# JayKickliter/Multirate.jl

Measured on AMD Instinct MI355X. Metric: Msamples/s in (Float32, 147//160, 24*147 taps) + achieved HBM GB/s vs roofline, higher is better.
Workload: dtype f32

## Files before the change

### multirate.jl_amd/csrc/api.hip

```cpp
#include <algorithm>
#include <cmath>
#include <chrono>
#include <cstdlib>
#include <cstring>
#include <mutex>
#include <numeric>
#include <unordered_map>

#include "mrhip_filter.h"

namespace mrhip {

bool plan_farrow_wave(const FarrowArgs &a);
hipError_t launch_farrow_wave(const TypeKey &tk, bool fused, const FarrowArgs &a, hipStream_t s, const char **kname, int num_cus);

thread_local LaunchEvents g_launch_events;
static thread_local std::string g_last_error;

void set_error(const std::string &msg) { g_last_error = msg; }

namespace {
struct OccKey { const void *fn; int dev; bool operator==(const OccKey &o) const { return fn == o.fn && dev == o.dev; } };
struct OccKeyHash { size_t operator()(const OccKey &k) const { return std::hash<const void *>()(k.fn) ^ (static_cast<size_t>(k.dev) * 0x9e3779b97f4a7c15ull); } };
struct OccEntry { unsigned block = 0; size_t lds = ~static_cast<size_t>(0), attr = 0; int per_cu = 0; };
// ... 1557 lines not shown
    }
    if (!same || stream_is_capturing(stream)) return single_calls();
    DeviceGuard guard(f0->device);
    if (!guard.ok) return fail(MRHIP_ERR_HIP, "hipSetDevice failed");
    const TypeKey tk = type_key(f0);
    const bool fused = f0->numerics == MRHIP_NUMERICS_FUSED;
    std::vector<CallPlan> plans(static_cast<size_t>(n));
    int64_t n_out_max = 0, nch_total = 0, x_len_max = 0;
    for (int i = 0; i < n; ++i) {
        mrhip_filter *f = filters[i];
        if (!f->mirror_valid)
            if (int rc = rec_pull(f)) return rc;
        plans[i] = plan_rational(f->kind, f->L, f->M, f->phiIdx, f->inputDeficit, x_len[i]);
        if (plans[i].n_out > y_capacity[i]) return fail(MRHIP_ERR_BUFFER_TOO_SMALL, "buffer is too small");
        n_out_max = std::max(n_out_max, plans[i].n_out);
        x_len_max = std::max(x_len_max, x_len[i]);
        nch_total += f->nch;
    }
    if (n_out_max < 1) return single_calls();
    PolyArgs a = poly_call_args(f0, x[0], y[0], x_len_max, n_out_max, x_len_max, false);
    a.n_out = n_out_max;
    a.u0 = 0; a.d0 = 1;
    a.nch = static_cast<int>(std::min<int64_t>(nch_total, 0x7fffffff));
    PairArgs pa;
    dim3 block;
    size_t lds = 0;
    const bool column = f0->L == 1;
    if (!(column ? plan_fir_stream(tk, a, f0->num_cus, &pa, &block, &lds) : plan_rational_opair(tk, fused, a, f0->num_cus, &pa, &block, &lds))) return single_calls();
    const size_t bytes = static_cast<size_t>(n) * sizeof(MultiDesc);
    if (int rc = multi_staging(f0, bytes)) return rc;
    MultiDesc *d = static_cast<MultiDesc *>(f0->multi_pin);
    unsigned steps_max = 0;
    for (int i = 0; i < n; ++i) {
        mrhip_filter *f = filters[i];
        if (int rc = adopt_stream(f, stream)) return rc;
        const CallPlan &p = plans[i];
        const int64_t spc = (p.n_out + pa.P - 1) / pa.P;
        if (spc * f->nch >= (1LL << 31)) return fail(MRHIP_ERR_INVALID_ARG, "stream too long for one launch");
        MultiDesc &m = d[i];
        m.x = x[i]; m.y = y[i]; m.hist = f->d_hist[f->hist_cur]; m.hist_new = f->d_hist[hist_other(f)]; m.taps = f->d_taps; m.rec = f->d_rec;
        m.x_stride = x_len[i]; m.y_stride = y_capacity[i]; m.x_len = x_len[i]; m.n_out = p.n_out;
        m.u0 = p.phi0 - 1; m.d0 = p.d0; m.phi_end = p.phi_end; m.d_end = p.d_end;
        m.steps_per_channel = static_cast<unsigned>(spc);
        m.total_steps = static_cast<unsigned>(spc * f->nch);
        m.spc_magic = step_magic(spc);
        m.nch = static_cast<int>(f->nch);
// ... 247 lines not shown
```

### multirate.jl_amd/csrc/kernels_rational_opair.hip

```cpp
#include <algorithm>
#include <cstdio>
#include <cstdlib>

#include "mrhip_internal.h"

namespace mrhip {

hipError_t launch_opair_f32_s0r(bool fused, int T, dim3 block, size_t lds, hipStream_t s, const PolyArgs &a, const PairArgs &pa, int num_cus);
hipError_t launch_opair_f32_s0c(bool fused, int T, dim3 block, size_t lds, hipStream_t s, const PolyArgs &a, const PairArgs &pa, int num_cus);
hipError_t launch_opair_f32_s1r(bool fused, int T, dim3 block, size_t lds, hipStream_t s, const PolyArgs &a, const PairArgs &pa, int num_cus);
hipError_t launch_opair_f32_s1c(bool fused, int T, dim3 block, size_t lds, hipStream_t s, const PolyArgs &a, const PairArgs &pa, int num_cus);
hipError_t launch_opair_f32_s0_long(int nc, bool fused, int T, dim3 block, size_t lds, hipStream_t s, const PolyArgs &a, const PairArgs &pa, int num_cus);
hipError_t launch_opair_f32_s1_long(int nc, bool fused, int T, dim3 block, size_t lds, hipStream_t s, const PolyArgs &a, const PairArgs &pa, int num_cus);
hipError_t launch_opair_f32_s2(int nc, bool fused, int T, dim3 block, size_t lds, hipStream_t s, const PolyArgs &a, const PairArgs &pa, int num_cus);
hipError_t launch_opair_f32_s3(int nc, bool fused, int T, dim3 block, size_t lds, hipStream_t s, const PolyArgs &a, const PairArgs &pa, int num_cus);
hipError_t launch_opair_f32_s4(int nc, bool fused, int T, dim3 block, size_t lds, hipStream_t s, const PolyArgs &a, const PairArgs &pa, int num_cus);
hipError_t launch_opair_f32_s5(int nc, bool fused, int T, dim3 block, size_t lds, hipStream_t s, const PolyArgs &a, const PairArgs &pa, int num_cus);
hipError_t launch_opair_wide_s0(bool x_f64, bool fused, int T, dim3 block, size_t lds, hipStream_t s, const PolyArgs &a, const PairArgs &pa, int num_cus);
hipError_t launch_opair_wide_s1(bool x_f64, bool fused, int T, dim3 block, size_t lds, hipStream_t s, const PolyArgs &a, const PairArgs &pa, int num_cus);
hipError_t launch_opair_cmix_s0(bool x_f64, bool fused, int T, dim3 block, size_t lds, hipStream_t s, const PolyArgs &a, const PairArgs &pa, int num_cus);
hipError_t launch_opair_cmix_s1(bool x_f64, bool fused, int T, dim3 block, size_t lds, hipStream_t s, const PolyArgs &a, const PairArgs &pa, int num_cus);

namespace {
constexpr int kOMaxThreads = 512;
#define opair_env_int(name, dflt) MRHIP_ENV_INT(name, dflt)
}

bool plan_rational_opair(const TypeKey &tk, bool fused, const PolyArgs &a, int num_cus, PairArgs *out, dim3 *block, size_t *lds, int force_wgpc)
{
    if (!opair_env_int("MRHIP_OPAIR", 1)) return false;
    if (tk.x_f64 && !tk.r_f64) return false;
    const int nc = tk.complex_x ? 2 : 1;
    const long long es = (tk.x_f64 ? 8 : 4) * nc;
#ifdef MRHIP_PS_FAST_BUILD
    if (a.T != 24 && !((a.T == 36 || a.T == 48) && !tk.complex_x) && !(!tk.r_f64 && (a.T == 36 || a.T == 48 || a.T == 56 || a.T == 64))) return false;
#endif
    if (a.T < 1 || a.T > (tk.r_f64 ? (tk.complex_x ? 32 : 48) : 64)) return false;
    if (a.L < 2 || a.M < 1 || a.zero_start_below > 0) return false;
    const int smin = static_cast<int>(a.M / a.L);
    if (smin > 5) return false;
    if (!opair_instantiated(fused, smin, a.T)) return false;
    if (smin >= 2 && (tk.r_f64 || a.T > 32)) return false;
    const int env_c = opair_env_int("MRHIP_OPAIR_C", 0), env_j = opair_env_int("MRHIP_OPAIR_J", 0), env_ns = opair_env_int("MRHIP_OPAIR_NS", 0);
    int best_c = 0;
    double best = -1.0;
    for (int pass = 0; pass < 2 && !best_c; ++pass)
        for (int c = 2; static_cast<long long>(c) * a.L / 2 <= kOMaxThreads && static_cast<long long>(c) * a.L <= 1024; c += 2) {
            const int lanes = static_cast<int>(static_cast<long long>(c) * a.L / 2);
            const int padded = (lanes + 63) / 64 * 64;
            if (pass == 0 && (padded < 192 || padded > 448)) continue;
            const double score = static_cast<double>(lanes) / padded * (padded < 192 ? 0.5 + 0.5 * padded / 192.0 : 1.0);
            if (score > best + 1e-9) { best = score; best_c = c; }
        }
    if (a.n_out * a.nch < (1LL << 22))
        for (int c = 2; static_cast<long long>(c) * a.L / 2 <= kOMaxThreads && static_cast<long long>(c) * a.L <= 1024; c += 2)
            if (static_cast<long long>(c) * a.L / 2 >= 128) { best_c = c; break; }
    if (env_c > 0 && env_c % 2 == 0 && static_cast<long long>(env_c) * a.L / 2 <= kOMaxThreads && static_cast<long long>(env_c) * a.L <= 1024) best_c = env_c;
    if (!best_c) return false;
    if (tk.r_f64 && a.T > 32 && (static_cast<long long>(best_c) * a.L / 2 + 63) / 64 > 7) return false;
    const int c = best_c;
    const long long cM = static_cast<long long>(c) * a.M, cL = static_cast<long long>(c) * a.L;
    const int lanes = static_cast<int>(cL / 2);
    const int padded = (lanes + 63) / 64 * 64;
    const int nwaves = padded / 64;
    const int tail = a.T + smin + 4;
    const int vgpr_est = (2 * a.T + (nc == 2 ? 36 : 30) + 7) / 8 * 8;
    const int waves_per_cu = tk.r_f64 ? 12 : 4 * std::min(8, 512 / vgpr_est);
    int wg_per_cu = std::max(1, std::min(4, waves_per_cu / (nwaves + 1)));
    if (nwaves + 1 == 6 && !tk.r_f64) wg_per_cu = 3;
    if (nwaves + 1 == 6 && tk.r_f64) wg_per_cu = 1;
    if (force_wgpc > 0) wg_per_cu = force_wgpc;
    if (const int env_w = opair_env_int("MRHIP_OPAIR_WGPC", 0); env_w > 0) wg_per_cu = env_w;
    int ns = env_ns >= 2 && env_ns <= 8 ? env_ns : (wg_per_cu == 1 ? 3 : 2);
    auto j_for = [&](int stages) -> long long {
        const long long budget_kib = ((wg_per_cu <= 3 ? 150 : 160) * 1024 / wg_per_cu - 64) / stages / 1024;
        const long long j = ((budget_kib > 1 ? budget_kib : 1) * 1024 / es - tail) / cM;
        return j < 1 ? 1 : j;
    };
    long long J = j_for(ns);
    if (env_j > 0) J = env_j;
    if (J > 64) J = 64;
    if (env_j <= 0) {
        const long long want_tiles = 4LL * num_cus;
        while (J > 2 && ((a.n_out + J * cL - 1) / (J * cL)) * a.nch < want_tiles) J = (J + 1) / 2;
    }
    const long long max_slots = 60 / (ns > 2 ? ns - 2 : 1);
    auto slots_for = [&](long long j) { return (((j * cM + tail + 3) / 4 * 4) * es / 16 + 63) / 64; };
    while (J > 1 && slots_for(J) > max_slots) --J;
    long long tile_len = (J * cM + tail + 3) / 4 * 4;
    const long long nslots = slots_for(J);
    const size_t stage_bytes = static_cast<size_t>(nslots) * 1024;
    if (nslots > max_slots || ns * stage_bytes > 156 * 1024) return false;
    PairArgs pa{};
    pa.c = c; pa.P = static_cast<int>(cL); pa.cM = static_cast<int>(cM);
    pa.Sout = pa.P; pa.lds_step = pa.cM; pa.run_chunks = 0; pa.q0 = 0; pa.run_magic = 0;
    pa.J = static_cast<int>(J);
    pa.tile_len = static_cast<int>(tile_len);
    pa.tail = tail;
    pa.dma_rounds = static_cast<int>(nslots);
    pa.stage_bytes = static_cast<int>(stage_bytes);
    pa.ns = ns;
    pa.nc = nc;
    pa.x_f64 = tk.x_f64 ? 1 : 0; pa.r_f64 = tk.r_f64 ? 1 : 0;
    pa.o0 = a.d0 - a.T;
    pa.tile_in = J * cM;
    pa.tile_out = J * cL;
    pa.tiles_per_channel = (a.n_out + pa.tile_out - 1) / pa.tile_out;
    pa.total_tiles = pa.tiles_per_channel * a.nch;
    if (a.n_out >= (1LL << 31) - pa.tile_out || pa.total_tiles >= (1LL << 31) - 65536) return false;
    const long long spc = (a.n_out + cL - 1) / cL;
    if (spc * a.nch >= (1LL << 31)) return false;
    pa.steps_per_channel = static_cast<unsigned>(spc);
    pa.total_steps = static_cast<unsigned>(spc * a.nch);
    pa.spc_magic = step_magic(spc);
    pa.flags_off = static_cast<int>(ns * stage_bytes);
    {
        const long long pt = (a.T + 4) | 1;
// ... 83 lines not shown
    *nblocks_out = nblocks;
    return true;
}

bool opair_ring_available(const TypeKey &tk, bool fused, const PolyArgs &a)
{
    if (fused || a.L < 2 || a.M < 1 || a.M / a.L > 1) return false;
    if (tk.x_f64 && !tk.r_f64) return false;
#ifdef MRHIP_PS_FAST_BUILD
    return a.T == 24;
#else
    return a.T == 24 || a.T == 32;
#endif
}

hipError_t launch_rational_opair(bool fused, const PolyArgs &a, const PairArgs &pa_in, dim3 block, size_t lds, hipStream_t s,
                                 const char **kname, int num_cus, unsigned *counters)
{
    if (!counters) return hipErrorInvalidValue;
    PairArgs pa = pa_in;
    pa.counters = counters;
    *kname = "rational_opair_kernel";
    const int smin = static_cast<int>(a.M / a.L);
    if (pa.r_f64 && pa.nc == 2)
        return smin == 0 ? launch_opair_cmix_s0(pa.x_f64 != 0, fused, a.T, block, lds, s, a, pa, num_cus)
                         : launch_opair_cmix_s1(pa.x_f64 != 0, fused, a.T, block, lds, s, a, pa, num_cus);
    if (pa.r_f64)
        return smin == 0 ? launch_opair_wide_s0(pa.x_f64 != 0, fused, a.T, block, lds, s, a, pa, num_cus)
                         : launch_opair_wide_s1(pa.x_f64 != 0, fused, a.T, block, lds, s, a, pa, num_cus);
    if (a.T > 48)
        return smin == 0 ? launch_opair_f32_s0_long(pa.nc, fused, a.T, block, lds, s, a, pa, num_cus) : launch_opair_f32_s1_long(pa.nc, fused, a.T, block, lds, s, a, pa, num_cus);
    switch (smin) {
    case 0: return pa.nc == 2 ? launch_opair_f32_s0c(fused, a.T, block, lds, s, a, pa, num_cus) : launch_opair_f32_s0r(fused, a.T, block, lds, s, a, pa, num_cus);
    case 1: return pa.nc == 2 ? launch_opair_f32_s1c(fused, a.T, block, lds, s, a, pa, num_cus) : launch_opair_f32_s1r(fused, a.T, block, lds, s, a, pa, num_cus);
    case 2: return launch_opair_f32_s2(pa.nc, fused, a.T, block, lds, s, a, pa, num_cus);
    case 3: return launch_opair_f32_s3(pa.nc, fused, a.T, block, lds, s, a, pa, num_cus);
    case 4: return launch_opair_f32_s4(pa.nc, fused, a.T, block, lds, s, a, pa, num_cus);
    case 5: return launch_opair_f32_s5(pa.nc, fused, a.T, block, lds, s, a, pa, num_cus);
    default: return hipErrorInvalidValue;
    }
}

}
```

### multirate.jl_amd/csrc/mrhip_internal.h

```cpp
#pragma once

#include <hip/hip_runtime.h>
#include <hip/hip_ext.h>

#include <cstdint>
#include <cstdlib>
#include <string>
#include <vector>

#include "multirate_hip.h"

namespace mrhip {

void set_error(const std::string &msg);
int fail(int code, const std::string &msg);

#define MRHIP_CHECK_HIP(expr)                                                                  \
    do {                                                                                       \
        hipError_t _e = (expr);                                                                \
        if (_e != hipSuccess)                                                                  \
            return ::mrhip::fail(MRHIP_ERR_HIP, std::string(#expr) + ": " + hipGetErrorString(_e)); \
    } while (0)

inline bool dtype_is_complex(int dt) { return dt == MRHIP_C64 || dt == MRHIP_C128; }
// ... 315 lines not shown

struct PairArgs {
    int c;
    int P;
    int cM;
    int J;
    int tile_len;
    int tail;
    int dma_rounds;
    int stage_bytes;
    int ns;
    int nc;
    int x_f64, r_f64;
    int ablate;
    unsigned steps_per_channel;
    unsigned total_steps;
    unsigned steps_per_group;
    int ngroups;
    int grid_cap;
    int flags_off;
    int pad_every;
    int bank_off;
    int static_grabs;
    int rt;
    int rt_rd;
    unsigned *counters;
    unsigned spc_magic;
    int Sout, lds_step, run_chunks, q0;
    unsigned run_magic;
    long long o0;
    long long tile_in;
    long long tile_out;
    long long tiles_per_channel;
    long long total_tiles;
    unsigned long long *probe;
};

constexpr size_t kCounterBytes = 33 * 256;

struct ArbTileArgs {
    int cpl;
    int tap_pitch;
    int bank_elems;
    int x_offset_bytes;
    int max_span;
    int prefetch;
// ... 43 lines not shown
{
    static const bool d = env_int_read("MRHIP_ENV_DYNAMIC", 0) != 0;
    return d;
}
#define MRHIP_ENV_INT(name, dflt) ([]() -> int { static const int v_ = ::mrhip::env_int_read(name, dflt); \
                                                 return ::mrhip::env_dynamic() ? ::mrhip::env_int_read(name, dflt) : v_; }())

struct TypeKey {
    bool x_f64;
    bool r_f64;
    bool complex_x;
};

hipError_t launch_poly_generic(const TypeKey &tk, bool fused, const PolyArgs &a, hipStream_t s, const char **kname);
hipError_t launch_arb_generic(const TypeKey &tk, bool fused, const ArbArgs &a, hipStream_t s, const char **kname);
hipError_t launch_farrow(const TypeKey &tk, bool fused, const FarrowArgs &a, hipStream_t s, const char **kname);
bool plan_farrow_tiled(const TypeKey &tk, const FarrowArgs &a, const int32_t *n_idx_host, const int *spans, int num_cus, ArbTileArgs *out, size_t *lds);
hipError_t launch_farrow_tiled(const TypeKey &tk, bool fused, const FarrowArgs &a, const ArbTileArgs &ta, size_t lds, hipStream_t s,
                               const char **kname, int num_cus);
hipError_t launch_shiftin(const TypeKey &tk, const HistArgs &a, hipStream_t s);
bool polyfit_rows(const double *y, int64_t n, int polyorder, double *coef);
bool plan_rational_opair(const TypeKey &tk, bool fused, const PolyArgs &a, int num_cus, PairArgs *out, dim3 *block, size_t *lds, int force_wgpc = 0);
bool plan_rational_opair_blocks(const TypeKey &tk, bool fused, const PolyArgs &a, int num_cus, PairArgs *out, dim3 *block, size_t *lds, int *nblocks);
hipError_t launch_rational_opair(bool fused, const PolyArgs &a, const PairArgs &pa, dim3 block, size_t lds, hipStream_t s,
                                 const char **kname, int num_cus, unsigned *counters);
constexpr bool opair_instantiated(bool fused, int smin, int T) { return !fused || (smin <= 1 && T % 4 == 0); }
bool plan_fir_stream(const TypeKey &tk, const PolyArgs &a, int num_cus, PairArgs *out, dim3 *block, size_t *lds);
hipError_t launch_fir_stream(bool fused, const PolyArgs &a, const PairArgs &pa, dim3 block, size_t lds, hipStream_t s,
                             const char **kname, int num_cus, unsigned *counters);
bool plan_arb_tiled(const TypeKey &tk, const ArbArgs &a, const int32_t *n_idx_host, const int *spans, int num_cus, ArbTileArgs *out, size_t *lds);
bool plan_arb_pipe(const TypeKey &tk, const ArbArgs &a, long long span256, ArbTileArgs *out, size_t *lds);
hipError_t launch_arb_pipe(const TypeKey &tk, bool fused, const ArbArgs &a, const ArbTileArgs &ta, size_t lds, hipStream_t s,
                           const char **kname, int num_cus);
struct ArbLaneArgs {
    int ring;
    int pitch8;
    int stretch;
    int chunk_max;
    int ngroups;
    int y16;
    unsigned *counters;
};
bool arb_lane_eligible(const TypeKey &tk, int T, int H, int64_t nch, double rate, int64_t x_len, int64_t x_stride, int64_t y_stride);
bool plan_arb_lane(const TypeKey &tk, const ArbArgs &a, double rate, ArbLaneArgs *out, size_t *lds);
hipError_t launch_arb_lane(bool fused, const ArbArgs &a, const ArbLaneArgs &la, size_t lds, hipStream_t s, const char **kname, int num_cus);
hipError_t launch_arb_tiled(const TypeKey &tk, bool fused, const ArbArgs &a, const ArbTileArgs &ta, size_t lds, hipStream_t s,
// ... 11 lines not shown
```

### multirate.jl_amd/csrc/opair_kernel.inc

```
#include <algorithm>
#include <cstdio>
#include <cstdlib>
#include <type_traits>
#include <vector>

#include "mrhip_internal.h"
#include "pair_device.h"
#include "pair_loader.h"

#pragma clang fp contract(off)

#ifndef MRHIP_OPAIR_WIDE_LONG
#define MRHIP_OPAIR_WIDE_LONG 1
#endif

namespace mrhip {
namespace {

constexpr int kOMaxThreads = 512;
constexpr int kOGroups = 32;

#define opair_env_int(name, dflt) MRHIP_ENV_INT(name, dflt)

using namespace dev;

__device__ __forceinline__ float fma_r(float a, float b, float c) { return __builtin_fmaf(a, b, c); }
__device__ __forceinline__ double fma_r(double a, double b, double c) { return __builtin_fma(a, b, c); }

template <bool FUSED, bool FIRST, bool COND, typename R>
__device__ __forceinline__ R slot_mac(R tap, R w, R acc, bool used)
{
    if constexpr (FIRST) {
        const R p = tap * w;
        if constexpr (COND) return used ? p : static_cast<R>(-0.0);
        else return p;
    } else if constexpr (FUSED) {
        const R r = fma_r(tap, w, acc);
        if constexpr (COND) return used ? r : acc;
        else return r;
    } else {
        R p = tap * w;
        if constexpr (COND) p = used ? p : static_cast<R>(-0.0);
        return acc + p;
    }
}

template <int T, bool FUSED, int NC, int SMIN, typename TXS, typename R, int MODE = 0>
#ifndef MRHIP_OPAIR_WIDE_WAVES
#define MRHIP_OPAIR_WIDE_WAVES 3
#endif
#ifndef MRHIP_RING_WAVES
#define MRHIP_RING_WAVES 4
#endif
__global__ __launch_bounds__(sizeof(R) == 8 && T > 32 ? kOMaxThreads : kOMaxThreads + 64, sizeof(R) == 8 ? (T > 32 ? 2 : MRHIP_OPAIR_WIDE_WAVES) : (MODE == 2 ? MRHIP_RING_WAVES : 3))
void rational_opair_kernel(PolyArgs a, PairArgs pa)
{
    constexpr unsigned ES = static_cast<unsigned>(sizeof(TXS)) * NC;
    constexpr unsigned OS = static_cast<unsigned>(sizeof(R)) * NC;
    constexpr int NW = static_cast<int>(ES / 4);
    static_assert(NW == 1 || NW == 2 || NW == 4, "sample size");
    using pair_t = std::conditional_t<NW == 1, v2u_t, v4u_t>;
    constexpr int SPRD = NW == 4 ? 1 : 2;
    constexpr int W = T + SMIN + 2;
    constexpr int NPR = (W + SPRD - 1) / SPRD;
    constexpr int NA = T + 1, NB = T + 2;

    extern __shared__ __attribute__((aligned(16))) unsigned char smem[];
    const unsigned lds_base = static_cast<unsigned>(reinterpret_cast<uintptr_t>(smem));
    const int tid = threadIdx.x;
    const int wave = __builtin_amdgcn_readfirstlane(tid >> 6), lane = tid & 63;
    const int ncw = (blockDim.x >> 6) - 1;
    constexpr bool RING = MODE == 2;
    if constexpr (MODE == 0) pair_take_dyn(a, pa);

    if (wave == ncw) {
        if constexpr (RING) pair_ring_loader_wave<NW, static_cast<int>(OS)>(a, pa, smem, lane);
        else pair_loader_wave<NW, MODE != 1>(a, pa, smem, lane);
        return;
    }
    if constexpr (RING) { if (blockIdx.x == 0) return; }
    volatile unsigned *const tile_flag = reinterpret_cast<volatile unsigned *>(smem + pa.flags_off);

    const int Li = static_cast<int>(a.L), Mi = static_cast<int>(a.M);
    int u0 = static_cast<int>(a.u0);
    const bool act = 2 * tid + 1 < pa.P;
    int uA = u0 + (act ? 2 * tid : 0) * Mi, uB = uA + Mi;
    int qA = uA / Li, phA = uA - qA * Li;
    int qB = uB / Li, phB = uB - qB * Li;
    int run0 = qA & ~1;
    int offA = qA - run0;
    int dB = qB - run0 - SMIN;
    R tapA[NA], tapB[NB];
    auto gather_taps = [&]() {
        const R *__restrict__ ca = static_cast<const R *>(a.taps) + static_cast<long long>(phA) * T;
        const R *__restrict__ cb = static_cast<const R *>(a.taps) + static_cast<long long>(phB) * T;
        R colA[T], colB[T];
#pragma unroll
        for (int i = 0; i < T; ++i) { colA[i] = ca[i]; colB[i] = cb[i]; }
#pragma unroll
        for (int j = 0; j < NA; ++j) {
            const R t0 = j < T ? colA[j] : R(0), t1 = j >= 1 ? colA[j - 1] : R(0);
            tapA[j] = act ? (offA == 0 ? t0 : t1) : R(0);
        }
#pragma unroll
        for (int j = 0; j < NB; ++j) {
            const R t0 = j < T ? colB[j] : R(0), t1 = (j >= 1 && j - 1 < T) ? colB[j - 1] : R(0), t2 = j >= 2 ? colB[j - 2] : R(0);
            tapB[j] = act ? (dB == 0 ? t0 : dB == 1 ? t1 : t2) : R(0);
        }
    };
    if constexpr (RING) {
#pragma unroll
        for (int j = 0; j < NA; ++j) tapA[j] = R(0);
#pragma unroll
        for (int j = 0; j < NB; ++j) tapB[j] = R(0);
        u0 = -1;
    } else if (pa.bank_off >= 0) {
        constexpr int PT = (T + 4) | 1;
        R *const bank = reinterpret_cast<R *>(smem + pa.bank_off);
        const R *__restrict__ tg = static_cast<const R *>(a.taps);
        const int ntaps = Li * T;
        for (int idx = tid; idx < ntaps; idx += ncw * 64) {
            const int col = idx / T, i = idx - col * T;
            bank[col * PT + 2 + i] = tg[idx];
        }
        asm volatile("s_waitcnt vmcnt(0) lgkmcnt(0)" ::: "memory");
        __builtin_amdgcn_s_barrier();
        const R *ba = bank + (act ? phA : 0) * PT + 2 - offA;
        const R *bb = bank + (act ? phB : 0) * PT + 2 - (act ? dB : 0);
#pragma unroll
        for (int j = 0; j < NA; ++j) tapA[j] = ba[j];
#pragma unroll
        for (int j = 0; j < NB; ++j) tapB[j] = bb[j];
#pragma unroll
        for (int j = 0; j < NA; ++j) pin(tapA[j]);
#pragma unroll
        for (int j = 0; j < NB; ++j) pin(tapB[j]);
    } else {
        const R *__restrict__ ca = static_cast<const R *>(a.taps) + static_cast<long long>(phA) * T;
        const R *__restrict__ cb = static_cast<const R *>(a.taps) + static_cast<long long>(phB) * T;
        R colA[T], colB[T];
#pragma unroll
        for (int i = 0; i < T; ++i) { colA[i] = ca[i]; colB[i] = cb[i]; }
#pragma unroll
        for (int j = 0; j < NA; ++j) {
            const R t0 = j < T ? colA[j] : R(0), t1 = j >= 1 ? colA[j - 1] : R(0);
            tapA[j] = act ? (offA == 0 ? t0 : t1) : R(0);
        }
#pragma unroll
        for (int j = 0; j < NB; ++j) {
            const R t0 = j < T ? colB[j] : R(0), t1 = (j >= 1 && j - 1 < T) ? colB[j - 1] : R(0), t2 = j >= 2 ? colB[j - 2] : R(0);
            tapB[j] = act ? (dB == 0 ? t0 : dB == 1 ? t1 : t2) : R(0);
        }
    }
    bool useA0 = offA == 0, useAT = offA == 1;
    bool useB0 = dB == 0, useB1 = dB <= 1, useBT = dB >= 1, useBT1 = dB == 2;

    const int n_out = static_cast<int>(a.n_out);
#ifdef MRHIP_OPAIR_PROBE
    unsigned long long pr_wait = 0, pr_tiles = 0;
    const unsigned long long pr_t0 = clock64(), pr_w0 = wall_clock64();
#endif
    unsigned ring_opts = 0;
    if constexpr (RING) ring_opts = static_cast<unsigned>(__builtin_amdgcn_readfirstlane(static_cast<int>(ld_sc1(&a.ring_dev->opts))));
    unsigned long long rs_bar = 0, rs_drain = 0;
    const unsigned long long rs_t0 = RING ? wall_clock64() : 0ull;
    bool pend = false;
    int p_stage = 0;
    unsigned p_slot = 0, p_shard = 0, p_cnt = 0, p_nshards = 0, p_seq_lo = 0, p_seq_hi = 0;
    for (int s = 0;; s = (s + 1 == pa.ns ? 0 : s + 1)) {
#ifdef MRHIP_OPAIR_PROBE
        const unsigned long long pr_a = clock64();
#endif
        unsigned long long rs_b0 = 0;
        if constexpr (RING) { if (ring_opts & 256u) rs_b0 = wall_clock64(); }
        __builtin_amdgcn_s_barrier();
        asm volatile("" ::: "memory");
        if constexpr (RING) { if (ring_opts & 256u) rs_bar += wall_clock64() - rs_b0; }
#ifdef MRHIP_OPAIR_PROBE
// ... 31 lines not shown
            if (u0_t != u0) {
                u0 = u0_t;
                uA = u0 + (act ? 2 * tid : 0) * Mi; uB = uA + Mi;
                qA = uA / Li; phA = uA - qA * Li;
                qB = uB / Li; phB = uB - qB * Li;
                run0 = qA & ~1; offA = qA - run0; dB = qB - run0 - SMIN;
                gather_taps();
                useA0 = offA == 0; useAT = offA == 1;
                useB0 = dB == 0; useB1 = dB <= 1; useBT = dB >= 1; useBT1 = dB == 2;
            }
        } else {
            const unsigned tg = static_cast<unsigned>(__builtin_amdgcn_readfirstlane(static_cast<int>(tile_flag[2 * s])));
            const unsigned tj = static_cast<unsigned>(__builtin_amdgcn_readfirstlane(static_cast<int>(tile_flag[2 * s + 1])));
            if (tj == 0u) break;
            const TileAt ta = pair_tile_at(pa, tg, tj);
            J = ta.jt;
            yc = static_cast<R *>(a.y) + (static_cast<long long>(ta.ch) * a.y_stride + static_cast<long long>(ta.st) * pa.Sout) * NC;
            remaining = n_out - ta.st * pa.Sout;
        }
        const bool full = remaining >= (J - 1) * pa.Sout + pa.P;
        unsigned lane_t;
        asm volatile("v_mbcnt_lo_u32_b32 %0, -1, 0\n\tv_mbcnt_hi_u32_b32 %0, -1, %0" : "=v"(lane_t));
        const unsigned tid_t = static_cast<unsigned>(wave) * 64u + lane_t;
        const unsigned my_out = 2u * tid_t;
        const unsigned uA_t = static_cast<unsigned>(u0) + (2u * tid_t < static_cast<unsigned>(pa.P) ? 2u * tid_t : 0u) * static_cast<unsigned>(Mi);
        const unsigned R_t = (uA_t / static_cast<unsigned>(Li)) & ~1u;
        const unsigned wbase = lds_base + static_cast<unsigned>(s) * pa.stage_bytes + (R_t - static_cast<unsigned>(pa.q0)) * ES;

        auto run_steps = [&](auto full_tag) {
            constexpr bool FULL = decltype(full_tag)::value;
            constexpr int KP = NPR < (NW == 1 ? 5 : 3) ? NPR : (NW == 1 ? 5 : 3);
            constexpr int NPRV = (NPR + KP - 1) / KP * KP;
            constexpr bool PAIRED_WAITS = KP >= 5;
            pair_t pring[KP];
            char *const ybytes = reinterpret_cast<char *>(yc);
            auto read_pair = [&](auto off_tag, unsigned addr) -> pair_t {
                constexpr int OFFP = decltype(off_tag)::value;
                if constexpr (NW == 1) return lds_read_b64<OFFP * 8>(addr);
                else return lds_read_b128<OFFP * 16>(addr);
            };
            static_for<0, KP>([&](auto I) { pring[decltype(I)::value] = read_pair(I, wbase); });
#pragma unroll 1
            for (int j = 0; j < J; ++j) {
                const int jn = j + 1 < J ? j + 1 : j;
                const unsigned wcur = wbase + static_cast<unsigned>(j) * pa.lds_step * ES;
                const unsigned wnext = wbase + static_cast<unsigned>(jn) * pa.lds_step * ES;
                R accA[NC] = {}, accB[NC] = {};
                static_for<0, NPRV>([&](auto I) {
                    constexpr int r = decltype(I)::value;
                    constexpr int slot = r % KP;
                    if constexpr (r < NPR) {
                        if constexpr (!PAIRED_WAITS) lgkm_wait<ring_younger(r, NPR, KP, 0)>(pring[slot]);
                        else if constexpr (r % 2 == 0) {
                            if constexpr (r + 1 < NPR) lgkm_wait2<ring_younger_pair(r, NPR, KP, 0)>(pring[slot], pring[(r + 1) % KP]);
                            else lgkm_wait<ring_younger(r, NPR, KP, 0)>(pring[slot]);
                        }
                        R wv[2][NC];
                        if constexpr (NW == 4) {
                            wv[0][0] = __hiloint2double(static_cast<int>(pring[slot].y), static_cast<int>(pring[slot].x));
                            wv[0][1] = __hiloint2double(static_cast<int>(pring[slot].w), static_cast<int>(pring[slot].z));
                        } else if constexpr (sizeof(TXS) == 8) {
                            wv[0][0] = __hiloint2double(static_cast<int>(pring[slot].y), static_cast<int>(pring[slot].x));
                            wv[1][0] = __hiloint2double(static_cast<int>(pring[slot].w), static_cast<int>(pring[slot].z));
                        } else if constexpr (NC == 1) {
                            wv[0][0] = static_cast<R>(__uint_as_float(pring[slot].x)); wv[1][0] = static_cast<R>(__uint_as_float(pring[slot].y));
                        } else {
                            wv[0][0] = static_cast<R>(__uint_as_float(pring[slot].x)); wv[0][1] = static_cast<R>(__uint_as_float(pring[slot].y));
                            wv[1][0] = static_cast<R>(__uint_as_float(pring[slot].z)); wv[1][1] = static_cast<R>(__uint_as_float(pring[slot].w));
                        }
                        static_for<0, SPRD>([&](auto H) {
                            constexpr int js = SPRD * r + decltype(H)::value;
                            constexpr int jb = js - SMIN;
                            constexpr bool a_lo = js < 1, a_hi = js > T - 1;
                            constexpr bool b_lo = jb < 2, b_hi = jb > T - 1;
#pragma unroll
                            for (int cc = 0; cc < NC; ++cc) {
                                const R w = wv[decltype(H)::value][cc];
                                if constexpr (js < NA) {
                                    const bool used = (a_lo ? useA0 : true) && (a_hi ? useAT : true);
                                    accA[cc] = slot_mac<FUSED, js == 0, a_lo || a_hi, R>(tapA[js], w, accA[cc], used);
                                }
                                if constexpr (jb >= 0 && jb < NB) {
                                    const bool used = (b_lo ? (jb == 0 ? useB0 : useB1) : true) && (b_hi ? (jb == T ? useBT : useBT1) : true);
                                    accB[cc] = slot_mac<FUSED, jb == 0, b_lo || b_hi, R>(tapB[jb], w, accB[cc], used);
                                }
                            }
                        });
#pragma unroll
                        for (int cc = 0; cc < NC; ++cc) { pin(accA[cc]); pin(accB[cc]); }
                    }
                    if constexpr (r + KP < NPR) pring[slot] = read_pair(std::integral_constant<int, r + KP>{}, wcur);
                    else if constexpr (r + KP >= NPRV) pring[slot] = read_pair(std::integral_constant<int, r + KP - NPRV>{}, wnext);
                });
                {
                    const unsigned kj = static_cast<unsigned>(j) * static_cast<unsigned>(pa.Sout);
                    char *const dst = ybytes + (kj + my_out) * OS;
                    R v[2 * NC];
#pragma unroll
                    for (int cc = 0; cc < NC; ++cc) { v[cc] = accA[cc]; v[NC + cc] = accB[cc]; }
                    auto put2 = [&]() { if constexpr (RING) { if (ring_nshards >> 31) { store_wt<2 * OS>(dst, v); return; } } __builtin_memcpy(dst, v, 2 * OS); };
                    auto put1 = [&]() { if constexpr (RING) { if (ring_nshards >> 31) { store_wt<OS>(dst, v); return; } } __builtin_memcpy(dst, v, OS); };
                    bool covered = false;
                    if constexpr (RING && 2 * OS == 8) {
                        if (!(ring_nshards >> 31)) {
                            covered = true;
                            const unsigned lim_x = FULL ? static_cast<unsigned>(pa.P) : (static_cast<unsigned>(remaining) > kj ? umin(static_cast<unsigned>(remaining) - kj, static_cast<unsigned>(pa.P)) : 0u);
                            if (my_out + 1 < lim_x) __builtin_memcpy(dst, v, 2 * OS);
                            else if (my_out < lim_x) __builtin_memcpy(dst, v, OS);
                        } else if (ring_opts & 8u) {
                            unsigned q[4];
                            q[0] = __float_as_uint(v[0]); q[1] = __float_as_uint(v[1]);
                            q[2] = static_cast<unsigned>(__builtin_amdgcn_mov_dpp(static_cast<int>(q[0]), 0xF5, 0xF, 0xF, false));
                            q[3] = static_cast<unsigned>(__builtin_amdgcn_mov_dpp(static_cast<int>(q[1]), 0xF5, 0xF, 0xF, false));
                            const unsigned lim_x = FULL ? static_cast<unsigned>(pa.P) : (static_cast<unsigned>(remaining) > kj ? umin(static_cast<unsigned>(remaining) - kj, static_cast<unsigned>(pa.P)) : 0u);
                            const bool even = (lane_t & 1u) == 0u;
                            if (even && my_out + 3 < lim_x) {
                                if (ring_opts & 2048u) {
// ... 73 lines not shown
inline void opair_probe_dump(unsigned long long *buf, long long g, hipStream_t s)
{
    if (!buf) return;
    (void)hipStreamSynchronize(s);
    std::vector<unsigned long long> h(static_cast<size_t>(g) * 8 * 4);
    (void)hipMemcpy(h.data(), buf, h.size() * 8, hipMemcpyDeviceToHost);
    if (FILE *f = std::fopen(std::getenv("MRHIP_PROBE_OUT"), "wb")) { std::fwrite(h.data(), 8, h.size(), f); std::fclose(f); }
}
#define MRHIP_PROBE_PRE(g) pa.probe = opair_probe_buf(g);
#define MRHIP_PROBE_POST(g) opair_probe_dump(pa.probe, g, s);
#else
#define MRHIP_PROBE_PRE(g)
#define MRHIP_PROBE_POST(g)
#endif

template <typename TXS, typename R>
constexpr bool opair_plain_instantiated(bool fused, int nc, int smin, int T)
{
    return !fused && smin <= 1 && (T == 24 || T == 32) && (nc >= 1) && sizeof(TXS) >= 4 && sizeof(R) >= 4;
}
template <bool FUSED, int NC, int SMIN, typename TXS, typename R>
hipError_t launch_opair_T(int T, dim3 block, size_t lds, hipStream_t s, const PolyArgs &a, PairArgs pa, int num_cus)
{
#define MRHIP_CASE(TT)                                                                              \
    case TT: if constexpr (opair_instantiated(FUSED, SMIN, TT)) {                                   \
        auto kfn = rational_opair_kernel<TT, FUSED, NC, SMIN, TXS, R>;                                       \
        if constexpr (opair_plain_instantiated<TXS, R>(FUSED, NC, SMIN, TT)) {                      \
            if (a.ring_dev) kfn = rational_opair_kernel<TT, FUSED, NC, SMIN, TXS, R, 2>;            \
                                                                                             \
            else if (!a.dyn && !a.multi && opair_env_int("MRHIP_OPAIR_PLAIN", 1))                                                           \
                kfn = a.n_out * a.nch >= (1LL << 22) ? rational_opair_kernel<TT, FUSED, NC, SMIN, TXS, R, 1> : rational_opair_kernel<TT, FUSED, NC, SMIN, TXS, R, 3>; \
        } else if (a.ring_dev) return hipErrorNotSupported;                                         \
        int per_cu = 0;                                                                             \
        hipError_t eo = occupancy_cached(reinterpret_cast<const void *>(kfn), block.x, lds, &per_cu); \
        if (eo != hipSuccess) return eo;                                                            \
        if (per_cu < 1) per_cu = 1;                                                                 \
        {    \
            const long long tiles = (static_cast<long long>(pa.total_steps) + pa.J - 1) / pa.J;     \
            if (block.x == 6 * 64 && per_cu > 3 && tiles > 3LL * num_cus * per_cu) per_cu = 3;      \
        }                                                                                           \
        const int bpc = opair_env_int("MRHIP_OPAIR_BPC", 0);                                 \
        if (bpc > 0) per_cu = bpc;                                                                  \
        long long g = static_cast<long long>(num_cus) * per_cu;                                     \
        if (g > static_cast<long long>(pa.total_steps)) g = pa.total_steps;                         \
        if (g < 1) g = 1;                                                                           \
        if (a.ring_dev) { g = static_cast<long long>(num_cus) * per_cu;    \
            if (pa.grid_cap > 1 && g > pa.grid_cap) g = pa.grid_cap; }                                  \
        pa.ngroups = static_cast<int>(g < kOGroups ? g : kOGroups);                                 \
        if (!a.ring_dev) pa.steps_per_group = static_cast<unsigned>((pa.total_steps + pa.ngroups - 1) / pa.ngroups);    \
        pa.static_grabs = (static_cast<long long>(pa.total_steps) + pa.J - 1) / pa.J <= 3 * g;      \
        if (a.multi) {    \
            long long w = static_cast<long long>(num_cus) * per_cu / a.multi_n;                     \
            const long long tiles = (static_cast<long long>(pa.total_steps) + pa.J - 1) / pa.J;     \
            if (w > tiles) w = tiles;                                                               \
            if (w < 1) w = 1;                                                                       \
            g = w * a.multi_n;                                                                      \
            pa.ngroups = a.multi_n;                                                                 \
            pa.static_grabs = 1;                                                                    \
        }                                                                                           \
        static int dbg = opair_env_int("MRHIP_DEBUG", 0);                                           \
        if (dbg == 1) {                                                                             \
            dbg = 0;                                                                                \
            hipFuncAttributes fa;                                                                   \
            (void)hipFuncGetAttributes(&fa, reinterpret_cast<const void *>(kfn));                   \
            std::fprintf(stderr, "[mrhip] rational_opair T=%d smin=%d in=%zuB arith=%zuB grid=%lld block=%u lds=%zu occ/CU=%d regs=%d c=%d P=%d cM=%d J=%d ns=%d\n", \
                         TT, SMIN, sizeof(TXS) * NC, sizeof(R), g, block.x, lds, per_cu, fa.numRegs, pa.c, pa.P, pa.cM, pa.J, pa.ns); \
        }                                                                                           \
        MRHIP_PROBE_PRE(g)                                                                          \
        launch_kernel(kfn, dim3(static_cast<unsigned>(g)), block, lds, s, a, pa);                   \
        MRHIP_PROBE_POST(g)                                                                         \
        return hipGetLastError();                                                                   \
    } else break;
#ifdef MRHIP_OPAIR_LONG
    switch (T) {
#ifdef MRHIP_PS_FAST_BUILD
        MRHIP_CASE(56) MRHIP_CASE(64)
#else
        MRHIP_CASE(49) MRHIP_CASE(50) MRHIP_CASE(51) MRHIP_CASE(52) MRHIP_CASE(53) MRHIP_CASE(54) MRHIP_CASE(55) MRHIP_CASE(56)
        MRHIP_CASE(57) MRHIP_CASE(58) MRHIP_CASE(59) MRHIP_CASE(60) MRHIP_CASE(61) MRHIP_CASE(62) MRHIP_CASE(63) MRHIP_CASE(64)
#endif
    default: break;
    }
#else
    switch (T) {
#ifdef MRHIP_PS_FAST_BUILD
        MRHIP_CASE(24)
#else
        MRHIP_CASE(1) MRHIP_CASE(2) MRHIP_CASE(3) MRHIP_CASE(4) MRHIP_CASE(5) MRHIP_CASE(6) MRHIP_CASE(7) MRHIP_CASE(8)
        MRHIP_CASE(9) MRHIP_CASE(10) MRHIP_CASE(11) MRHIP_CASE(12) MRHIP_CASE(13) MRHIP_CASE(14) MRHIP_CASE(15) MRHIP_CASE(16)
        MRHIP_CASE(17) MRHIP_CASE(18) MRHIP_CASE(19) MRHIP_CASE(20) MRHIP_CASE(21) MRHIP_CASE(22) MRHIP_CASE(23) MRHIP_CASE(24)
        MRHIP_CASE(25) MRHIP_CASE(26) MRHIP_CASE(27) MRHIP_CASE(28) MRHIP_CASE(29) MRHIP_CASE(30) MRHIP_CASE(31) MRHIP_CASE(32)
#endif
    default: break;
    }
    if constexpr ((sizeof(R) == 4 || (NC == 1 && MRHIP_OPAIR_WIDE_LONG)) && SMIN <= 1) {
        switch (T) {
#ifndef MRHIP_PS_FAST_BUILD
        MRHIP_CASE(33) MRHIP_CASE(34) MRHIP_CASE(35) MRHIP_CASE(36) MRHIP_CASE(37) MRHIP_CASE(38) MRHIP_CASE(39) MRHIP_CASE(40)
        MRHIP_CASE(41) MRHIP_CASE(42) MRHIP_CASE(43) MRHIP_CASE(44) MRHIP_CASE(45) MRHIP_CASE(46) MRHIP_CASE(47) MRHIP_CASE(48)
#else
        MRHIP_CASE(36) MRHIP_CASE(48)
#endif
        default: break;
        }
    }
#endif
    return hipErrorInvalidValue;
#undef MRHIP_CASE
}

}
}
```

Baseline: 656,100.

## Add four-outputs-per-lane variant of the rational opair kernel for Float32

Adds a kernel instantiation in which each lane computes four consecutive output samples instead of two, reusing the staged input window from LDS across more outputs and halving the lane count per tile. The planner now picks a quad form for large plain Float32 real streams with T of 24 or 32 and M below 2L, and changes the lane, tail and register estimates to match. It also marks multi-filter batches so they stay on the two-output path. The quad form roughly doubles tap registers per lane, which can lower occupancy, and it adds more involved partial-tile store logic.

New measurement: 648,900 (median of 2 runs). -1.1%, worse.

```diff
diff --git a/multirate.jl_amd/csrc/api.hip b/multirate.jl_amd/csrc/api.hip
--- a/multirate.jl_amd/csrc/api.hip
+++ b/multirate.jl_amd/csrc/api.hip
@@ -1603,6 +1603,7 @@
     a.n_out = n_out_max;
     a.u0 = 0; a.d0 = 1;
     a.nch = static_cast<int>(std::min<int64_t>(nch_total, 0x7fffffff));
+    a.multi_n = n;
     PairArgs pa;
     dim3 block;
     size_t lds = 0;
diff --git a/multirate.jl_amd/csrc/kernels_rational_opair.hip b/multirate.jl_amd/csrc/kernels_rational_opair.hip
--- a/multirate.jl_amd/csrc/kernels_rational_opair.hip
+++ b/multirate.jl_amd/csrc/kernels_rational_opair.hip
@@ -20,10 +20,25 @@
 hipError_t launch_opair_wide_s1(bool x_f64, bool fused, int T, dim3 block, size_t lds, hipStream_t s, const PolyArgs &a, const PairArgs &pa, int num_cus);
 hipError_t launch_opair_cmix_s0(bool x_f64, bool fused, int T, dim3 block, size_t lds, hipStream_t s, const PolyArgs &a, const PairArgs &pa, int num_cus);
 hipError_t launch_opair_cmix_s1(bool x_f64, bool fused, int T, dim3 block, size_t lds, hipStream_t s, const PolyArgs &a, const PairArgs &pa, int num_cus);
+hipError_t launch_opair_f32_quad(int smin, int T, dim3 block, size_t lds, hipStream_t s, const PolyArgs &a, const PairArgs &pa, int num_cus);
 
 namespace {
 constexpr int kOMaxThreads = 512;
 #define opair_env_int(name, dflt) MRHIP_ENV_INT(name, dflt)
+}
+
+bool opair_quad_eligible(bool fused, int nc, bool x_f64, bool r_f64, const PolyArgs &a)
+{
+    if (!opair_env_int("MRHIP_OPAIR_QUAD", 1) || !opair_env_int("MRHIP_OPAIR_PLAIN", 1)) return false;
+    if (fused || nc != 1 || x_f64 || r_f64) return false;
+#ifdef MRHIP_PS_FAST_BUILD
+    if (a.T != 24) return false;
+#else
+    if (a.T != 24 && a.T != 32) return false;
+#endif
+    if (a.dyn || a.multi || a.multi_n > 0 || a.ring_dev) return false;
+    if (a.L < 2 || a.M < 1 || a.M >= 2 * a.L || 3 * (a.M % a.L) > a.L) return false;
+    return a.n_out * a.nch >= (1LL << 22);
 }
 
 bool plan_rational_opair(const TypeKey &tk, bool fused, const PolyArgs &a, int num_cus, PairArgs *out, dim3 *block, size_t *lds, int force_wgpc)
@@ -42,32 +57,41 @@
     if (!opair_instantiated(fused, smin, a.T)) return false;
     if (smin >= 2 && (tk.r_f64 || a.T > 32)) return false;
     const int env_c = opair_env_int("MRHIP_OPAIR_C", 0), env_j = opair_env_int("MRHIP_OPAIR_J", 0), env_ns = opair_env_int("MRHIP_OPAIR_NS", 0);
+    bool quad = force_wgpc == 0 && opair_quad_eligible(fused, nc, tk.x_f64, tk.r_f64, a);
     int best_c = 0;
-    double best = -1.0;
-    for (int pass = 0; pass < 2 && !best_c; ++pass)
-        for (int c = 2; static_cast<long long>(c) * a.L / 2 <= kOMaxThreads && static_cast<long long>(c) * a.L <= 1024; c += 2) {
-            const int lanes = static_cast<int>(static_cast<long long>(c) * a.L / 2);
-            const int padded = (lanes + 63) / 64 * 64;
-            if (pass == 0 && (padded < 192 || padded > 448)) continue;
-            const double score = static_cast<double>(lanes) / padded * (padded < 192 ? 0.5 + 0.5 * padded / 192.0 : 1.0);
-            if (score > best + 1e-9) { best = score; best_c = c; }
-        }
-    if (a.n_out * a.nch < (1LL << 22))
-        for (int c = 2; static_cast<long long>(c) * a.L / 2 <= kOMaxThreads && static_cast<long long>(c) * a.L <= 1024; c += 2)
-            if (static_cast<long long>(c) * a.L / 2 >= 128) { best_c = c; break; }
-    if (env_c > 0 && env_c % 2 == 0 && static_cast<long long>(env_c) * a.L / 2 <= kOMaxThreads && static_cast<long long>(env_c) * a.L <= 1024) best_c = env_c;
+    for (int form = 0; form < 2 && !best_c; ++form) {
+        if (form == 1) { if (!quad) break; quad = false; }
+        const int opl = quad ? 4 : 2;
+        const long long max_p = quad ? 2048 : 1024;
+        auto c_ok = [&](int c) { return static_cast<long long>(c) * a.L / opl <= kOMaxThreads && static_cast<long long>(c) * a.L <= max_p && static_cast<long long>(c) * a.L % opl == 0; };
+        double best = -1.0;
+        for (int pass = 0; pass < 2 && !best_c; ++pass)
+            for (int c = 2; static_cast<long long>(c) * a.L / opl <= kOMaxThreads && static_cast<long long>(c) * a.L <= max_p; c += 2) {
+                if (!c_ok(c)) continue;
+                const int lanes = static_cast<int>(static_cast<long long>(c) * a.L / opl);
+                const int padded = (lanes + 63) / 64 * 64;
+                if (pass == 0 && (padded < 192 || padded > 448)) continue;
+                const double score = static_cast<double>(lanes) / padded * (padded < 192 ? 0.5 + 0.5 * padded / 192.0 : 1.0);
+                if (score > best + 1e-9) { best = score; best_c = c; }
+            }
+        if (a.n_out * a.nch < (1LL << 22))
+            for (int c = 2; static_cast<long long>(c) * a.L / 2 <= kOMaxThreads && static_cast<long long>(c) * a.L <= 1024; c += 2)
+                if (static_cast<long long>(c) * a.L / 2 >= 128) { best_c = c; break; }
+        if (env_c > 0 && env_c % 2 == 0 && c_ok(env_c)) best_c = env_c;
+    }
     if (!best_c) return false;
+    const int opl = quad ? 4 : 2;
     if (tk.r_f64 && a.T > 32 && (static_cast<long long>(best_c) * a.L / 2 + 63) / 64 > 7) return false;
     const int c = best_c;
     const long long cM = static_cast<long long>(c) * a.M, cL = static_cast<long long>(c) * a.L;
-    const int lanes = static_cast<int>(cL / 2);
+    const int lanes = static_cast<int>(cL / opl);
     const int padded = (lanes + 63) / 64 * 64;
     const int nwaves = padded / 64;
-    const int tail = a.T + smin + 4;
-    const int vgpr_est = (2 * a.T + (nc == 2 ? 36 : 30) + 7) / 8 * 8;
+    const int tail = a.T + (opl - 1) * smin + 4;
+    const int vgpr_est = ((quad ? 4 * a.T + 37 : 2 * a.T + (nc == 2 ? 36 : 30)) + 7) / 8 * 8;
     const int waves_per_cu = tk.r_f64 ? 12 : 4 * std::min(8, 512 / vgpr_est);
     int wg_per_cu = std::max(1, std::min(4, waves_per_cu / (nwaves + 1)));
-    if (nwaves + 1 == 6 && !tk.r_f64) wg_per_cu = 3;
+    if (nwaves + 1 == 6 && !tk.r_f64) wg_per_cu = quad ? 1 : 3;
     if (nwaves + 1 == 6 && tk.r_f64) wg_per_cu = 1;
     if (force_wgpc > 0) wg_per_cu = force_wgpc;
     if (const int env_w = opair_env_int("MRHIP_OPAIR_WGPC", 0); env_w > 0) wg_per_cu = env_w;
@@ -93,6 +117,7 @@
     if (nslots > max_slots || ns * stage_bytes > 156 * 1024) return false;
     PairArgs pa{};
     pa.c = c; pa.P = static_cast<int>(cL); pa.cM = static_cast<int>(cM);
+    pa.opl = opl;
     pa.Sout = pa.P; pa.lds_step = pa.cM; pa.run_chunks = 0; pa.q0 = 0; pa.run_magic = 0;
     pa.J = static_cast<int>(J);
     pa.tile_len = static_cast<int>(tile_len);
@@ -222,6 +247,8 @@
     pa.counters = counters;
     *kname = "rational_opair_kernel";
     const int smin = static_cast<int>(a.M / a.L);
+    if (pa.opl == 4)
+        return opair_quad_eligible(fused, pa.nc, pa.x_f64 != 0, pa.r_f64 != 0, a) ? launch_opair_f32_quad(smin, a.T, block, lds, s, a, pa, num_cus) : hipErrorInvalidValue;
     if (pa.r_f64 && pa.nc == 2)
         return smin == 0 ? launch_opair_cmix_s0(pa.x_f64 != 0, fused, a.T, block, lds, s, a, pa, num_cus)
                          : launch_opair_cmix_s1(pa.x_f64 != 0, fused, a.T, block, lds, s, a, pa, num_cus);
diff --git a/multirate.jl_amd/csrc/kernels_rational_opair_f32_quad.hip b/multirate.jl_amd/csrc/kernels_rational_opair_f32_quad.hip
--- /dev/null
+++ b/multirate.jl_amd/csrc/kernels_rational_opair_f32_quad.hip
@@ -0,0 +1,13 @@
+#define MRHIP_OPAIR_QUAD_UNIT
+#include "opair_kernel.inc"
+
+namespace mrhip {
+
+hipError_t launch_opair_f32_quad(int smin, int T, dim3 block, size_t lds, hipStream_t s, const PolyArgs &a, const PairArgs &pa, int num_cus)
+{
+    if (a.dyn || a.multi || a.ring_dev || pa.opl != 4) return hipErrorInvalidValue;
+    return smin == 0 ? launch_opair_T<false, 1, 0, float, float>(T, block, lds, s, a, pa, num_cus)
+                     : launch_opair_T<false, 1, 1, float, float>(T, block, lds, s, a, pa, num_cus);
+}
+
+}
diff --git a/multirate.jl_amd/csrc/mrhip_internal.h b/multirate.jl_amd/csrc/mrhip_internal.h
--- a/multirate.jl_amd/csrc/mrhip_internal.h
+++ b/multirate.jl_amd/csrc/mrhip_internal.h
@@ -361,6 +361,7 @@
     int pad_every;
     int bank_off;
     int static_grabs;
+    int opl;
     int rt;
     int rt_rd;
     unsigned *counters;
@@ -450,6 +451,7 @@
 bool polyfit_rows(const double *y, int64_t n, int polyorder, double *coef);
 bool plan_rational_opair(const TypeKey &tk, bool fused, const PolyArgs &a, int num_cus, PairArgs *out, dim3 *block, size_t *lds, int force_wgpc = 0);
 bool plan_rational_opair_blocks(const TypeKey &tk, bool fused, const PolyArgs &a, int num_cus, PairArgs *out, dim3 *block, size_t *lds, int *nblocks);
+bool opair_quad_eligible(bool fused, int nc, bool x_f64, bool r_f64, const PolyArgs &a);
 hipError_t launch_rational_opair(bool fused, const PolyArgs &a, const PairArgs &pa, dim3 block, size_t lds, hipStream_t s,
                                  const char **kname, int num_cus, unsigned *counters);
 constexpr bool opair_instantiated(bool fused, int smin, int T) { return !fused || (smin <= 1 && T % 4 == 0); }
diff --git a/multirate.jl_amd/csrc/opair_kernel.inc b/multirate.jl_amd/csrc/opair_kernel.inc
--- a/multirate.jl_amd/csrc/opair_kernel.inc
+++ b/multirate.jl_amd/csrc/opair_kernel.inc
@@ -45,7 +45,7 @@
     }
 }
 
-template <int T, bool FUSED, int NC, int SMIN, typename TXS, typename R, int MODE = 0>
+template <int T, bool FUSED, int NC, int SMIN, typename TXS, typename R, int MODE = 0, int OPL = 2>
 #ifndef MRHIP_OPAIR_WIDE_WAVES
 #define MRHIP_OPAIR_WIDE_WAVES 3
 #endif
@@ -61,7 +61,8 @@
     static_assert(NW == 1 || NW == 2 || NW == 4, "sample size");
     using pair_t = std::conditional_t<NW == 1, v2u_t, v4u_t>;
     constexpr int SPRD = NW == 4 ? 1 : 2;
-    constexpr int W = T + SMIN + 2;
+    static_assert(OPL == 2 || (OPL == 4 && MODE == 1 && !FUSED && NC == 1 && sizeof(TXS) == 4 && sizeof(R) == 4 && SMIN <= 1), "four outputs per lane: PLAIN, STRICT, Float32 real");
+    constexpr int W = T + (OPL - 1) * SMIN + 2;
     constexpr int NPR = (W + SPRD - 1) / SPRD;
     constexpr int NA = T + 1, NB = T + 2;
 
@@ -83,14 +84,22 @@
 
     const int Li = static_cast<int>(a.L), Mi = static_cast<int>(a.M);
     int u0 = static_cast<int>(a.u0);
-    const bool act = 2 * tid + 1 < pa.P;
-    int uA = u0 + (act ? 2 * tid : 0) * Mi, uB = uA + Mi;
+    const bool act = OPL * tid + (OPL - 1) < pa.P;
+    int uA = u0 + (act ? OPL * tid : 0) * Mi, uB = uA + Mi;
     int qA = uA / Li, phA = uA - qA * Li;
     int qB = uB / Li, phB = uB - qB * Li;
     int run0 = qA & ~1;
     int offA = qA - run0;
     int dB = qB - run0 - SMIN;
     R tapA[NA], tapB[NB];
+    int phC = 0, phD = 0, dC = 0, dD = 0;
+    R tapC[NB], tapD[NB];
+    if constexpr (OPL == 4) {
+        const int uC = uB + Mi, uD = uC + Mi;
+        const int qC = uC / Li, qD = uD / Li;
+        phC = uC - qC * Li; phD = uD - qD * Li;
+        dC = qC - run0 - 2 * SMIN; dD = qD - run0 - 3 * SMIN;
+    }
     auto gather_taps = [&]() {
         const R *__restrict__ ca = static_cast<const R *>(a.taps) + static_cast<long long>(phA) * T;
         const R *__restrict__ cb = static_cast<const R *>(a.taps) + static_cast<long long>(phB) * T;
@@ -131,10 +140,20 @@
         for (int j = 0; j < NA; ++j) tapA[j] = ba[j];
 #pragma unroll
         for (int j = 0; j < NB; ++j) tapB[j] = bb[j];
+        if constexpr (OPL == 4) {
+            const R *bc = bank + (act ? phC : 0) * PT + 2 - (act ? dC : 0);
+            const R *bd = bank + (act ? phD : 0) * PT + 2 - (act ? dD : 0);
+#pragma unroll
+            for (int j = 0; j < NB; ++j) { tapC[j] = bc[j]; tapD[j] = bd[j]; }
+        }
 #pragma unroll
         for (int j = 0; j < NA; ++j) pin(tapA[j]);
 #pragma unroll
         for (int j = 0; j < NB; ++j) pin(tapB[j]);
+        if constexpr (OPL == 4) {
+#pragma unroll
+            for (int j = 0; j < NB; ++j) { pin(tapC[j]); pin(tapD[j]); }
+        }
     } else {
         const R *__restrict__ ca = static_cast<const R *>(a.taps) + static_cast<long long>(phA) * T;
         const R *__restrict__ cb = static_cast<const R *>(a.taps) + static_cast<long long>(phB) * T;
@@ -151,9 +170,28 @@
             const R t0 = j < T ? colB[j] : R(0), t1 = (j >= 1 && j - 1 < T) ? colB[j - 1] : R(0), t2 = j >= 2 ? colB[j - 2] : R(0);
             tapB[j] = act ? (dB == 0 ? t0 : dB == 1 ? t1 : t2) : R(0);
         }
+        if constexpr (OPL == 4) {
+            auto column = [&](R (&tap)[NB], int ph, int d) {
+                const R *__restrict__ cg = static_cast<const R *>(a.taps) + static_cast<long long>(ph) * T;
+                R col[T];
+#pragma unroll
+                for (int i = 0; i < T; ++i) col[i] = cg[i];
+#pragma unroll
+                for (int j = 0; j < NB; ++j) {
+                    const R t0 = j < T ? col[j] : R(0), t1 = (j >= 1 && j - 1 < T) ? col[j - 1] : R(0), t2 = j >= 2 ? col[j - 2] : R(0);
+                    tap[j] = act ? (d == 0 ? t0 : d == 1 ? t1 : t2) : R(0);
+                }
+#pragma unroll
+                for (int j = 0; j < NB; ++j) pin(tap[j]);
+            };
+            column(tapC, phC, dC);
+            column(tapD, phD, dD);
+        }
     }
     bool useA0 = offA == 0, useAT = offA == 1;
     bool useB0 = dB == 0, useB1 = dB <= 1, useBT = dB >= 1, useBT1 = dB == 2;
+    const bool useC0 = dC == 0, useC1 = dC <= 1, useCT = dC >= 1, useCT1 = dC == 2;
+    const bool useD0 = dD == 0, useD1 = dD <= 1, useDT = dD >= 1, useDT1 = dD == 2;
 
     const int n_out = static_cast<int>(a.n_out);
 #ifdef MRHIP_OPAIR_PROBE
@@ -231,8 +269,8 @@
         unsigned lane_t;
         asm volatile("v_mbcnt_lo_u32_b32 %0, -1, 0\n\tv_mbcnt_hi_u32_b32 %0, -1, %0" : "=v"(lane_t));
         const unsigned tid_t = static_cast<unsigned>(wave) * 64u + lane_t;
-        const unsigned my_out = 2u * tid_t;
-        const unsigned uA_t = static_cast<unsigned>(u0) + (2u * tid_t < static_cast<unsigned>(pa.P) ? 2u * tid_t : 0u) * static_cast<unsigned>(Mi);
+        const unsigned my_out = static_cast<unsigned>(OPL) * tid_t;
+        const unsigned uA_t = static_cast<unsigned>(u0) + (my_out < static_cast<unsigned>(pa.P) ? my_out : 0u) * static_cast<unsigned>(Mi);
         const unsigned R_t = (uA_t / static_cast<unsigned>(Li)) & ~1u;
         const unsigned wbase = lds_base + static_cast<unsigned>(s) * pa.stage_bytes + (R_t - static_cast<unsigned>(pa.q0)) * ES;
 
@@ -255,6 +293,7 @@
                 const unsigned wcur = wbase + static_cast<unsigned>(j) * pa.lds_step * ES;
                 const unsigned wnext = wbase + static_cast<unsigned>(jn) * pa.lds_step * ES;
                 R accA[NC] = {}, accB[NC] = {};
+                R accC = R(0), accD = R(0);
                 static_for<0, NPRV>([&](auto I) {
                     constexpr int r = decltype(I)::value;
                     constexpr int slot = r % KP;
@@ -293,15 +332,45 @@
                                     const bool used = (b_lo ? (jb == 0 ? useB0 : useB1) : true) && (b_hi ? (jb == T ? useBT : useBT1) : true);
                                     accB[cc] = slot_mac<FUSED, jb == 0, b_lo || b_hi, R>(tapB[jb], w, accB[cc], used);
                                 }
+                                if constexpr (OPL == 4) {
+                                    constexpr int jc = js - 2 * SMIN, jd = js - 3 * SMIN;
+                                    if constexpr (jc >= 0 && jc < NB) {
+                                        constexpr bool lo = jc < 2, hi = jc > T - 1;
+                                        const bool used = (lo ? (jc == 0 ? useC0 : useC1) : true) && (hi ? (jc == T ? useCT : useCT1) : true);
+                                        accC = slot_mac<FUSED, jc == 0, lo || hi, R>(tapC[jc], w, accC, used);
+                                    }
+                                    if constexpr (jd >= 0 && jd < NB) {
+                                        constexpr bool lo = jd < 2, hi = jd > T - 1;
+                                        const bool used = (lo ? (jd == 0 ? useD0 : useD1) : true) && (hi ? (jd == T ? useDT : useDT1) : true);
+                                        accD = slot_mac<FUSED, jd == 0, lo || hi, R>(tapD[jd], w, accD, used);
+                                    }
+                                }
                             }
                         });
 #pragma unroll
                         for (int cc = 0; cc < NC; ++cc) { pin(accA[cc]); pin(accB[cc]); }
+                        if constexpr (OPL == 4) { pin(accC); pin(accD); }
                     }
                     if constexpr (r + KP < NPR) pring[slot] = read_pair(std::integral_constant<int, r + KP>{}, wcur);
                     else if constexpr (r + KP >= NPRV) pring[slot] = read_pair(std::integral_constant<int, r + KP - NPRV>{}, wnext);
                 });
-                {
+                if constexpr (OPL == 4) {
+                    const unsigned kj = static_cast<unsigned>(j) * static_cast<unsigned>(pa.Sout);
+                    char *const dst = ybytes + (kj + my_out) * OS;
+                    const R v[4] = {accA[0], accB[0], accC, accD};
+                    if constexpr (FULL) {
+                        if (my_out + 3 < static_cast<unsigned>(pa.P)) __builtin_memcpy(dst, v, 4 * OS);
+                    } else {
+                        const unsigned rem_j = static_cast<unsigned>(remaining) > kj ? static_cast<unsigned>(remaining) - kj : 0u;
+                        const unsigned lim = rem_j < static_cast<unsigned>(pa.P) ? rem_j : static_cast<unsigned>(pa.P);
+                        if (my_out + 3 < lim) __builtin_memcpy(dst, v, 4 * OS);
+                        else {
+                            if (my_out + 1 < lim) __builtin_memcpy(dst, v, 2 * OS);
+                            else if (my_out < lim) __builtin_memcpy(dst, v, OS);
+                            if (my_out + 2 < lim) __builtin_memcpy(dst + 2 * OS, v + 2, OS);
+                        }
+                    }
+                } else {
                     const unsigned kj = static_cast<unsigned>(j) * static_cast<unsigned>(pa.Sout);
                     char *const dst = ybytes + (kj + my_out) * OS;
                     R v[2 * NC];
@@ -421,10 +490,17 @@
 template <bool FUSED, int NC, int SMIN, typename TXS, typename R>
 hipError_t launch_opair_T(int T, dim3 block, size_t lds, hipStream_t s, const PolyArgs &a, PairArgs pa, int num_cus)
 {
+#ifdef MRHIP_OPAIR_QUAD_UNIT
+#define MRHIP_OPAIR_KFN0(TT) rational_opair_kernel<TT, FUSED, NC, SMIN, TXS, R, 1, 4>
+#define MRHIP_OPAIR_MODES(TT) false
+#else
+#define MRHIP_OPAIR_KFN0(TT) rational_opair_kernel<TT, FUSED, NC, SMIN, TXS, R>
+#define MRHIP_OPAIR_MODES(TT) opair_plain_instantiated<TXS, R>(FUSED, NC, SMIN, TT)
+#endif
 #define MRHIP_CASE(TT)                                                                              \
     case TT: if constexpr (opair_instantiated(FUSED, SMIN, TT)) {                                   \
-        auto kfn = rational_opair_kernel<TT, FUSED, NC, SMIN, TXS, R>;                                       \
-        if constexpr (opair_plain_instantiated<TXS, R>(FUSED, NC, SMIN, TT)) {                      \
+        auto kfn = MRHIP_OPAIR_KFN0(TT);                                                            \
+        if constexpr (MRHIP_OPAIR_MODES(TT)) {                                                      \
             if (a.ring_dev) kfn = rational_opair_kernel<TT, FUSED, NC, SMIN, TXS, R, 2>;            \
                                                                                              \
             else if (!a.dyn && !a.multi && opair_env_int("MRHIP_OPAIR_PLAIN", 1))                                                           \
@@ -462,15 +538,23 @@
             dbg = 0;                                                                                \
             hipFuncAttributes fa;                                                                   \
             (void)hipFuncGetAttributes(&fa, reinterpret_cast<const void *>(kfn));                   \
-            std::fprintf(stderr, "[mrhip] rational_opair T=%d smin=%d in=%zuB arith=%zuB grid=%lld block=%u lds=%zu occ/CU=%d regs=%d c=%d P=%d cM=%d J=%d ns=%d\n", \
-                         TT, SMIN, sizeof(TXS) * NC, sizeof(R), g, block.x, lds, per_cu, fa.numRegs, pa.c, pa.P, pa.cM, pa.J, pa.ns); \
+            std::fprintf(stderr, "[mrhip] rational_opair T=%d smin=%d in=%zuB arith=%zuB grid=%lld block=%u lds=%zu occ/CU=%d regs=%d c=%d P=%d cM=%d J=%d ns=%d opl=%d\n", \
+                         TT, SMIN, sizeof(TXS) * NC, sizeof(R), g, block.x, lds, per_cu, fa.numRegs, pa.c, pa.P, pa.cM, pa.J, pa.ns, pa.opl == 4 ? 4 : 2); \
         }                                                                                           \
         MRHIP_PROBE_PRE(g)                                                                          \
         launch_kernel(kfn, dim3(static_cast<unsigned>(g)), block, lds, s, a, pa);                   \
         MRHIP_PROBE_POST(g)                                                                         \
         return hipGetLastError();                                                                   \
     } else break;
-#ifdef MRHIP_OPAIR_LONG
+#if defined(MRHIP_OPAIR_QUAD_UNIT)
+    switch (T) {
+        MRHIP_CASE(24)
+#ifndef MRHIP_PS_FAST_BUILD
+        MRHIP_CASE(32)
+#endif
+    default: break;
+    }
+#elif defined(MRHIP_OPAIR_LONG)
     switch (T) {
 #ifdef MRHIP_PS_FAST_BUILD
         MRHIP_CASE(56) MRHIP_CASE(64)
@@ -506,7 +590,9 @@
 #endif
     return hipErrorInvalidValue;
 #undef MRHIP_CASE
-}
-
-}
-}
+#undef MRHIP_OPAIR_KFN0
+#undef MRHIP_OPAIR_MODES
+}
+
+}
+}
```
